# anonymousauthors001/SGS-GNN

Hardware: AMD Instinct MI355X
Metric: sampled edges/sec + training steps/sec, Reddit hybrid 20% sparsity (higher is better)
Workload: dtype f32

## Files before the change

include/sgs_hip.h:

```cpp
#ifndef SGS_HIP_H_
#define SGS_HIP_H_

#include <stddef.h>
#include <stdint.h>

#ifdef __cplusplus
extern "C" {
#endif

#define SGS_ABI_VERSION 1

#define SGS_OK 0
#define SGS_EINVAL (-1)
#define SGS_EWORKSPACE (-2)
#define SGS_EHIP (-3)

typedef void* sgs_stream_t;

int sgs_abi_version(void);
const char* sgs_last_error(void);

int sgs_rng_set_epoch_buffer(const uint64_t* epoch_dev);
int sgs_exp_noise(uint64_t seed, uint64_t stream_id, int64_t E, float* noise, sgs_stream_t stream);
int sgs_dropout_keep(uint64_t seed, uint32_t site, int64_t rows, int64_t cols, float p, uint8_t* keep,
// ... 481 lines not shown
    void* ws;
    size_t ws_bytes;
} SgsGemmTnProblem;
int sgs_gemm_tn_group_supported(int64_t K, int64_t M, int64_t N);
int sgs_gemm_tn_group(const SgsGemmTnProblem* problems, int count, sgs_stream_t stream);

int sgs_er_weight(const int64_t* edge_index, int64_t E, int64_t N, const int32_t* out_ptr, const int32_t* out_dst, int walk_lengths,
                  int walks, uint64_t seed, float* weight, sgs_stream_t stream);

int sgs_adam_max_tensors(void);
int sgs_adam_step(const int64_t* desc_host, int64_t n_tensors, float lr, float beta1, float beta2, float eps, float weight_decay,
                  int maximize, uint32_t* ticket, sgs_stream_t stream);
int sgs_adam_multi_max_tensors(void);
int sgs_adam_step_multi(const int64_t* desc_host, const float* hyper_host, int64_t n_tensors, uint32_t* ticket, float* loss_sum, const float* loss,
                        uint64_t* epoch, sgs_stream_t stream);

size_t sgs_sample_topq_multi_workspace_bytes(int64_t E, int64_t D);
int sgs_sample_topq_multi(int mode, const float* p, const float* prior, double degree_bias_coef, const float* noise, uint64_t seed,
                          uint64_t stream_id0, int64_t D, int64_t E, int64_t q, const int64_t* edge_index, uint8_t* mask, int64_t* sampled_eid,
                          int64_t* sampled_edge_index, float* stats, float* st_weights, void* ws, size_t ws_bytes, sgs_stream_t stream);
size_t sgs_sample_topq_multi_cover_workspace_bytes(int64_t E, int64_t N, int64_t D);
int sgs_sample_topq_multi_cover_group_set(int G);
int sgs_sample_topq_multi_cover(int mode, const float* p, const float* prior, double degree_bias_coef, const float* noise, uint64_t seed,
                                uint64_t stream_id0, int64_t D, int64_t E, int64_t q, const int64_t* edge_index, int64_t N,
                                const int32_t* in_ptr, const int32_t* in_src, const int32_t* in_eid, uint8_t* mask, int64_t* sampled_eid,
                                int64_t* sampled_edge_index, float* stats, float* st_weights, int32_t* cover_info, void* ws, size_t ws_bytes,
                                sgs_stream_t stream);
size_t sgs_graph_filter_multi_workspace_bytes(int64_t E_parent, int64_t N, int64_t D);
int sgs_graph_filter_multi(const int32_t* pin_ptr, const int32_t* pin_src, const int32_t* pin_eid, int64_t E_parent, int64_t N, int64_t D,
                           const uint8_t* mask, const int64_t* sampled_eid, int64_t q, int32_t* in_ptr, int32_t* in_src, int32_t* in_eid,
// ... 82 lines not shown
```

sgs-gnn_amd/csrc/gemm_tn.hip:

```cpp
#include "sgs_common.h"

namespace sgs {
namespace {

using f32x16 = __attribute__((ext_vector_type(16))) float;
constexpr int kUnroll = 8;

__global__ void __launch_bounds__(64) gemm_tn_tile(const float* __restrict__ A, const float* __restrict__ B, int64_t K, int M, int N,
                                                  int ksplit, float* __restrict__ slab) {
    const int lane = threadIdx.x, kh = lane >> 5, l31 = lane & 31;
    const int ti = blockIdx.x, tj = blockIdx.y, s = blockIdx.z;
    const int i = ti * 32 + l31, j = tj * 32 + l31;
    const bool iok = i < M, jok = j < N;
    const int64_t per = ((K + ksplit - 1) / ksplit + 1) & ~int64_t(1);
    const int64_t k0 = s * per, k1 = (k0 + per < K) ? k0 + per : K;
    f32x16 acc;
#pragma unroll
    for (int r = 0; r < 16; ++r) acc[r] = 0.f;
    int64_t k = k0;
    for (; k + 2 * kUnroll <= k1; k += 2 * kUnroll) {
        float a[kUnroll], b[kUnroll];
#pragma unroll
        for (int u = 0; u < kUnroll; ++u) {
            const int64_t kk = k + 2 * u + kh;
// ... 8 lines not shown
        const float a = (iok && kk < k1) ? A[kk * M + i] : 0.f;
        const float b = (jok && kk < k1) ? B[kk * N + j] : 0.f;
        acc = __builtin_amdgcn_mfma_f32_32x32x2f32(a, b, acc, 0, 0, 0);
    }
    float* out = slab + static_cast<int64_t>(s) * M * N;
    if (jok) {
#pragma unroll
        for (int r = 0; r < 16; ++r) {
            const int row = ti * 32 + (r & 3) + 8 * (r >> 2) + 4 * kh;
            if (row < M) out[static_cast<int64_t>(row) * N + j] = acc[r];
        }
    }
}

constexpr int kWgUnroll = 8;
template <int NW>
__device__ __forceinline__ void gemm_tn_wg_tile(const float* __restrict__ A, const float* __restrict__ B, int64_t K, int M, int N,
                                                float* __restrict__ C, int64_t ldc, int ti, int tj) {
    __shared__ float red[NW][16][64];
    const int lane = threadIdx.x & 63, s = threadIdx.x >> 6, kh = lane >> 5, l31 = lane & 31;
    const int i = ti * 32 + l31, j = tj * 32 + l31;
    const bool iok = i < M, jok = j < N;
    const int64_t per = ((K + NW - 1) / NW + 1) & ~int64_t(1);
    const int64_t k0 = s * per, k1 = (k0 + per < K) ? k0 + per : K;
    f32x16 acc;
#pragma unroll
    for (int r = 0; r < 16; ++r) acc[r] = 0.f;
    int64_t k = k0;
    for (; k + 2 * kWgUnroll <= k1; k += 2 * kWgUnroll) {
        float a[kWgUnroll], b[kWgUnroll];
#pragma unroll
        for (int u = 0; u < kWgUnroll; ++u) {
            const int64_t kk = k + 2 * u + kh;
            a[u] = iok ? A[kk * M + i] : 0.f;
// ... 7 lines not shown
        const float a = (iok && kk < k1) ? A[kk * M + i] : 0.f;
        const float b = (jok && kk < k1) ? B[kk * N + j] : 0.f;
        acc = __builtin_amdgcn_mfma_f32_32x32x2f32(a, b, acc, 0, 0, 0);
    }
#pragma unroll
    for (int r = 0; r < 16; ++r) red[s][r][lane] = acc[r];
    __syncthreads();
    if (!jok) return;
    constexpr int RPW = 16 / NW;
#pragma unroll
    for (int q = 0; q < RPW; ++q) {
        const int r = s * RPW + q;
        float sum = 0.f;
#pragma unroll
        for (int z = 0; z < NW; ++z) sum += red[z][r][lane];
        const int row = ti * 32 + (r & 3) + 8 * (r >> 2) + 4 * kh;
        if (row < M) C[static_cast<int64_t>(row) * ldc + j] = sum;
    }
}

template <int NW>
__global__ void __launch_bounds__(64 * NW) gemm_tn_wg(const float* __restrict__ A, const float* __restrict__ B, int64_t K, int M, int N,
                                                     float* __restrict__ C, int64_t ldc) {
    gemm_tn_wg_tile<NW>(A, B, K, M, N, C, ldc, blockIdx.x, blockIdx.y);
}

constexpr int kGroupMax = 8;
struct GemmTnDesc {
    const float* A;
    const float* B;
    float* C;
    int64_t K, ldc;
    int M, N;
    int first_tile, tiles_i;
};
struct GemmTnGroupArgs {
    GemmTnDesc d[kGroupMax];
    int count;
};

template <int NW>
__global__ void __launch_bounds__(64 * NW) gemm_tn_wg_group(GemmTnGroupArgs a) {
    const int t = static_cast<int>(blockIdx.x);
    int pi = 0;
    while (pi + 1 < a.count && t >= a.d[pi + 1].first_tile) ++pi;
    const GemmTnDesc& d = a.d[pi];
    const int local = t - d.first_tile;
    const int tj = local / d.tiles_i, ti = local - tj * d.tiles_i;
    gemm_tn_wg_tile<NW>(d.A, d.B, d.K, d.M, d.N, d.C, d.ldc, ti, tj);
}

__global__ void __launch_bounds__(256) gemm_tn_reduce(const float* __restrict__ slab, int64_t mn, int ksplit, float* __restrict__ C,
                                                      const float* __restrict__ cpart = nullptr, int M = 0, float* __restrict__ colsum = nullptr,
                                                      int N = 0, int64_t ldc = 0, const float* __restrict__ rowscale = nullptr,
                                                      float scale = 1.f, const float* __restrict__ dzpart = nullptr, int nz = 0,
                                                      float* __restrict__ dzsum = nullptr, float* __restrict__ Craw = nullptr,
                                                      float* __restrict__ csraw = nullptr, int csplit = 0) {
    const int64_t i = static_cast<int64_t>(blockIdx.x) * 256 + threadIdx.x;
    if (i >= mn) {
        const int64_t c = i - mn;
        if (dzsum && c == M) {
            float acc = 0.f;
            for (int z = 0; z < nz; ++z) acc += dzpart[z];
            dzsum[0] = acc;
// ... 877 lines not shown
        else              hipLaunchKernelGGL((gemm_tn_wg<2>), grid, dim3(128), 0, stream, A, B, K, static_cast<int>(M), static_cast<int>(N), C, ld);
        SGS_LAUNCH_OK();
        return SGS_OK;
    } else
        hipLaunchKernelGGL(gemm_tn_tile, dim3(cdiv(M, 32), cdiv(N, 32), ks), dim3(64), 0, stream, A, B, K, static_cast<int>(M),
                           static_cast<int>(N), ks, dst);
    if (ks > 1 || strided)
        hipLaunchKernelGGL(gemm_tn_reduce, dim3(cdiv(M * N + (colsum_A ? M : 0), 256)), dim3(256), 0, stream, slab, M * N, n_slabs, C,
                           static_cast<const float*>(colsum_A ? cpart : nullptr), static_cast<int>(M), colsum_A, static_cast<int>(N), ldc);
    SGS_LAUNCH_OK();
    return SGS_OK;
}

int sgs_gemm_tn_group_supported(int64_t K, int64_t M, int64_t N) { return wg_waves(K, M, N); }

int sgs_gemm_tn_group(const SgsGemmTnProblem* problems, int count, sgs_stream_t stream_) {
    hipStream_t stream = static_cast<hipStream_t>(stream_);
    SGS_REQUIRE(count >= 0 && (count == 0 || problems), SGS_EINVAL, "sgs_gemm_tn_group: bad problem list");
    for (int p = 0; p < count; ++p) {
        const SgsGemmTnProblem& q = problems[p];
        SGS_REQUIRE(q.K >= 0 && q.M >= 0 && q.N >= 0 && q.M < (1 << 30) && q.N < (1 << 30), SGS_EINVAL, "sgs_gemm_tn_group: bad sizes");
        SGS_REQUIRE(q.ldc == 0 || q.ldc >= q.N, SGS_EINVAL, "sgs_gemm_tn_group: ldc < N");
        SGS_REQUIRE(q.M == 0 || q.N == 0 || (q.C && (q.K == 0 || (q.A && q.B))), SGS_EINVAL, "sgs_gemm_tn_group: null pointer");
    }
    for (int nw = 16; nw >= 2; nw >>= 1) {
        GemmTnGroupArgs a;
        a.count = 0;
        int tiles = 0;
        auto flush = [&]() {
            if (a.count == 0) return;
            for (int z = a.count; z < kGroupMax; ++z) a.d[z] = a.d[0];
            const dim3 grid(static_cast<unsigned>(tiles));
// ... 16 lines not shown
            tiles += d.tiles_i * static_cast<int>(cdiv(q.N, 32));
            if (a.count == kGroupMax) flush();
        }
        flush();
    }
    SGS_LAUNCH_OK();
    for (int p = 0; p < count; ++p) {
        const SgsGemmTnProblem& q = problems[p];
        if (wg_waves(q.K, q.M, q.N) != 0) continue;
        const int rc = gemm_tn_impl(q.A, q.B, q.K, q.M, q.N, q.C, nullptr, q.ws, q.ws_bytes, stream, q.ldc);
        if (rc != SGS_OK) return rc;
    }
    return SGS_OK;
}

}
```

sgs-gnn_amd/csrc/optim.hip:

```cpp
#include "sgs_common.h"

namespace sgs {
namespace {

constexpr int kAT = 256;
constexpr int kAChunk = 2048;
constexpr int kAMax = 24;

struct AdamDesc {
    float* p;
    const float* g;
    float* m;
    float* v;
    int64_t n;
    float* step;
    const float* gate;
};
struct AdamArgs {
    AdamDesc d[kAMax];
    int chunk_end[kAMax];
    int n_tensors;
    float lr, beta1, beta2, eps, weight_decay;
    int maximize;
    unsigned int* ticket;
};

__global__ void __launch_bounds__(kAT) adam_group(AdamArgs a) {
    __shared__ unsigned int s_last;
    int ti = 0;
    while (static_cast<int>(blockIdx.x) >= a.chunk_end[ti]) ++ti;
    const int chunk = static_cast<int>(blockIdx.x) - (ti ? a.chunk_end[ti - 1] : 0);
    const AdamDesc d = a.d[ti];
    const bool open = d.gate == nullptr || d.gate[0] != 0.f;
    const float t = d.step[0] + 1.0f;
    const double bc1 = 1.0 - exp(static_cast<double>(t) * log(static_cast<double>(a.beta1)));
    const double bc2 = 1.0 - exp(static_cast<double>(t) * log(static_cast<double>(a.beta2)));
    const float step_size = static_cast<float>(static_cast<double>(a.lr) / bc1);
    const float inv_sqrt_bc2 = static_cast<float>(1.0 / sqrt(bc2));
    const float beta1 = a.beta1, beta2 = a.beta2, eps = a.eps, wd = a.weight_decay;
    const int64_t base = static_cast<int64_t>(chunk) * kAChunk;
#pragma unroll
    for (int it = 0; it < kAChunk / kAT; ++it) {
        const int64_t i = base + static_cast<int64_t>(it) * kAT + threadIdx.x;
        if (open && i < d.n) {
            float g = d.g[i];
            if (a.maximize) g = -g;
            const float p = d.p[i];
            if (wd != 0.f) g = fmaf(wd, p, g);
            float m = d.m[i], v = d.v[i];
            m = m + (g - m) * (1.0f - beta1);
            v = beta2 * v + (1.0f - beta2) * g * g;
            const float denom = sqrtf(v) * inv_sqrt_bc2 + eps;
            d.m[i] = m;
            d.v[i] = v;
            d.p[i] = p - step_size * (m / denom);
        }
    }
    __syncthreads();
    if (threadIdx.x == 0) s_last = (atomicAdd(a.ticket, 1u) == gridDim.x - 1) ? 1u : 0u;
    __syncthreads();
    if (s_last) {
        if (static_cast<int>(threadIdx.x) < a.n_tensors) {
            const AdamDesc& dd = a.d[threadIdx.x];
            if (dd.gate == nullptr || dd.gate[0] != 0.f) dd.step[0] += 1.0f;
        }
        if (threadIdx.x == 0) __hip_atomic_store(a.ticket, 0u, __ATOMIC_RELAXED, __HIP_MEMORY_SCOPE_AGENT);
    }
}

constexpr int kAMax2 = 16;
struct AdamState {
    float* m;
    float* v;
    float* step;
    const float* gate;
    float lr, beta1, beta2, eps, wd;
    int maximize;
};
struct AdamDesc2 {
    float* p;
    const float* g;
    int64_t n;
    AdamState s[2];
    int n_states;
};
struct AdamArgs2 {
    AdamDesc2 d[kAMax2];
    int chunk_end[kAMax2];
    int n_tensors;
    unsigned int* ticket;
    float* loss_sum;
    const float* loss;
    unsigned long long* epoch;
};

__global__ void __launch_bounds__(kAT) adam_multi(AdamArgs2 a) {
    __shared__ unsigned int s_last;
    int ti = 0;
    while (static_cast<int>(blockIdx.x) >= a.chunk_end[ti]) ++ti;
    const int chunk = static_cast<int>(blockIdx.x) - (ti ? a.chunk_end[ti - 1] : 0);
    const AdamDesc2& d = a.d[ti];
    bool open[2];
    float step_size[2], inv_sqrt_bc2[2];
#pragma unroll
    for (int q = 0; q < 2; ++q) {
        open[q] = q < d.n_states && (d.s[q].gate == nullptr || d.s[q].gate[0] != 0.f);
        step_size[q] = 0.f;
        inv_sqrt_bc2[q] = 0.f;
        if (q < d.n_states) {
            const float t = d.s[q].step[0] + 1.0f;
            const double bc1 = 1.0 - exp(static_cast<double>(t) * log(static_cast<double>(d.s[q].beta1)));
            const double bc2 = 1.0 - exp(static_cast<double>(t) * log(static_cast<double>(d.s[q].beta2)));
            step_size[q] = static_cast<float>(static_cast<double>(d.s[q].lr) / bc1);
            inv_sqrt_bc2[q] = static_cast<float>(1.0 / sqrt(bc2));
        }
    }
    const int64_t base = static_cast<int64_t>(chunk) * kAChunk;
#pragma unroll
    for (int it = 0; it < kAChunk / kAT; ++it) {
        const int64_t i = base + static_cast<int64_t>(it) * kAT + threadIdx.x;
        if (i < d.n && (open[0] || open[1])) {
            const float g0 = d.g[i];
            float p = d.p[i];
#pragma unroll
            for (int q = 0; q < 2; ++q) {
                if (open[q]) {
                    const AdamState& st = d.s[q];
                    float g = st.maximize ? -g0 : g0;
                    if (st.wd != 0.f) g = fmaf(st.wd, p, g);
                    float m = st.m[i], v = st.v[i];
                    m = m + (g - m) * (1.0f - st.beta1);
                    v = st.beta2 * v + (1.0f - st.beta2) * g * g;
                    const float denom = sqrtf(v) * inv_sqrt_bc2[q] + st.eps;
                    st.m[i] = m;
                    st.v[i] = v;
                    p = p - step_size[q] * (m / denom);
                }
            }
            d.p[i] = p;
        }
    }
    __syncthreads();
    if (threadIdx.x == 0) s_last = (atomicAdd(a.ticket, 1u) == gridDim.x - 1) ? 1u : 0u;
    __syncthreads();
    if (s_last) {
        if (static_cast<int>(threadIdx.x) < 2 * a.n_tensors) {
            const AdamDesc2& dd = a.d[threadIdx.x >> 1];
            const int q = threadIdx.x & 1;
            if (q < dd.n_states && (dd.s[q].gate == nullptr || dd.s[q].gate[0] != 0.f)) {
                dd.s[q].step[0] += 1.0f;
            }
        }
        if (threadIdx.x == 64) {
            if (a.loss_sum && a.loss) a.loss_sum[0] += a.loss[0];
            if (a.epoch) a.epoch[0] += 1ull;
// ... 98 lines not shown
```

sgs-gnn_amd/ops.py:

```python
from __future__ import annotations

import ctypes
import os
from typing import NamedTuple, Optional

import numpy as np
import torch

from . import _lib

SAMPLE_LEARNED, SAMPLE_PRIOR = 0, 1
ACT_NONE, ACT_RELU, ACT_RELU_DROPOUT = 0, 1, 2

_workspaces = {}
_retired_workspaces = []
_pin_workspaces = False


def _need_gpu(*tensors):
    for t in tensors:
        if t is not None and not t.is_cuda:
            raise RuntimeError("sgs_gnn_amd: the SGS hot path runs only on a HIP device (got a CPU tensor); "
                               "there is no CPU fallback")

# ... 93 lines not shown


def new_memo_scope() -> int:
    global _memo_scope
    _memo_scope += 1
    return _memo_scope


def drop_memos(module) -> None:
    for mod in module.modules():
        if getattr(mod, "_lin_cache", None) is not None:
            mod._lin_cache = None


GEMM_TN_LAUNCHES = {"single": 0, "group": 0}
_defer = None
_defer_enabled = True


def set_deferred_weight_grads(on: bool) -> None:
    global _defer_enabled
    _defer_enabled = bool(on)


class deferred_weight_grads:

    def __init__(self, *roots):
        self.roots = roots
        self.producers, self.queue, self.armed, self.prev = {}, [], False, None

    def __enter__(self):
        global _defer
        self.prev = _defer
        if not _defer_enabled:
            return self
        seen, stack = set(), [r.grad_fn for r in self.roots if r.grad_fn is not None]
        prod = self.producers = {}
        while stack:
            fn = stack.pop()
            if fn in seen:
                continue
            seen.add(fn)
            for nxt, _ in fn.next_functions:
                if nxt is None:
# ... 22 lines not shown
        p = node.variable
        if p.grad is not None or getattr(p, "_backward_hooks", None) or getattr(p, "_post_accumulate_grad_hooks", None):
            return None
        return node

    def _enqueue(self, node, dY, x, grad, c_ptr, K, M, N, ldc):
        if not self.armed:
            torch.autograd.Variable._execution_engine.queue_callback(self._flush)
            self.armed = True
        self.queue.append((node, dY, x, grad.data_ptr(), c_ptr, K, M, N, ldc, grad.device.index))

    def _flush(self):
        q, self.queue, self.armed = self.queue, [], False
        if not q:
            return
        L = _lib.lib()
        for node, _, _, base, *_ in q:
            g = node.variable.grad
            if g is None or g.data_ptr() != base:
                raise RuntimeError("sgs_gnn_amd: a deferred weight gradient did not become its parameter's .grad as it was (the values "
                                   "autograd passed on were read before they were written)")
        words = []
        for _, dY, x, _, c_ptr, K, M, N, ldc, _ in q:
            words += [dY.data_ptr(), x.data_ptr(), K, M, N, c_ptr, ldc, 0, 0]
        arr = (ctypes.c_int64 * len(words))(*words)
        dev = q[0][9]
        stream = _raw_stream(dev) if _raw_stream is not None else torch.cuda.current_stream(dev).cuda_stream
        GEMM_TN_LAUNCHES["group"] += 1
        _lib.check(L.sgs_gemm_tn_group(arr, len(q), stream), "sgs_gemm_tn_group")


def _leaf_dw(dY, x, K, M, N, leaf=None, out=None, col0=0):
    L = _lib.lib()
    dW = out if out is not None else torch.empty(M, N, dtype=torch.float32, device=x.device)
    ldc = dW.shape[1]
    c_ptr = _ptr(dW) + 4 * col0
    dY_p, x_p = _ptr(dY, torch.float32), _ptr(x, torch.float32)
    if _defer is not None and leaf is not None and L.sgs_gemm_tn_group_supported(K, M, N) > 0:
        node = _defer._leaf_slot_ok(*leaf)
        if node is not None:
            _defer._enqueue(node, dY, x, dW, c_ptr, K, M, N, ldc)
            return dW
    ws = workspace(L.sgs_gemm_tn_workspace_bytes(K, M, N), x.device)
    GEMM_TN_LAUNCHES["single"] += 1
# ... 2715 lines not shown
```

sgs-gnn_amd/optim.py:

```python
from __future__ import annotations

import ctypes

import torch

from . import _lib, ops


class FusedAdam(torch.optim.Optimizer):
    def __init__(self, params, lr=1e-3, betas=(0.9, 0.999), eps=1e-8, weight_decay=0.0, maximize=False):
        if lr < 0 or eps < 0 or not (0 <= betas[0] < 1) or not (0 <= betas[1] < 1) or weight_decay < 0:
            raise ValueError("FusedAdam: invalid hyper-parameters")
        defaults = dict(lr=lr, betas=betas, eps=eps, weight_decay=weight_decay, maximize=maximize, capturable=True, amsgrad=False,
                        foreach=None, fused=None, differentiable=False)
        super().__init__(params, defaults)
        self._tickets = {}
        self._ticket_pool = None

    def _init_state(self, p):
        if self._ticket_pool is None:
            self._ticket_pool = torch.zeros(64, dtype=torch.int32, device=p.device)
        st = self.state[p]
        if len(st) == 0:
            st["step"] = torch.zeros((), dtype=torch.float32, device=p.device)
# ... 37 lines not shown
                    if self._ticket_pool is not None and len(self._tickets) < self._ticket_pool.numel():
                        i = len(self._tickets)
                        tk = self._tickets[key] = self._ticket_pool[i:i + 1]
                    else:
                        tk = self._tickets[key] = torch.zeros(1, dtype=torch.int32, device=part[0].device)
                arr = (ctypes.c_int64 * len(words))(*words)
                _lib.check(L.sgs_adam_step(arr, len(part), float(group["lr"]), float(b1), float(b2), float(group["eps"]),
                                           float(group["weight_decay"]), int(bool(group["maximize"])), tk.data_ptr(), stream),
                           "sgs_adam_step")
                if not torch.cuda.is_current_stream_capturing():
                    torch.autograd.graph.increment_version(part)
        return loss

    @staticmethod
    @torch.no_grad()
    def step_many(optimizers, tick=None):
        opts = list(optimizers)
        L = _lib.lib()
        order, states = [], {}
        for o in opts:
            if not isinstance(o, FusedAdam):
                raise RuntimeError("FusedAdam.step_many: every optimiser must be a FusedAdam")
            for group in o.param_groups:
                for p in group["params"]:
                    if p.grad is None:
                        continue
                    if id(p) not in states:
                        states[id(p)] = []
                        order.append(p)
                    states[id(p)].append((o, group))
        if any(len(v) > 2 for v in states.values()):
            for o in opts:
                o.step()
            if tick is not None:
                ops.loss_tick(*tick)
            return
        tick_ptrs = (None, None, None)
        if tick is not None:
            loss_sum, loss, epoch = tick
            tick_ptrs = (loss_sum.data_ptr(), loss.detach().reshape(1).data_ptr(), epoch.data_ptr())
        kmax = L.sgs_adam_multi_max_tensors()
        stream = ops._stream()
        first = opts[0]
        if not order:
            if tick is not None:
                ops.loss_tick(*tick)
            return
        for lo in range(0, len(order), kmax):
            part = order[lo:lo + kmax]
            words, hyper = [], []
            for p in part:
                g = p.grad
                if (p.dtype != torch.float32 or g.dtype != torch.float32 or not p.is_cuda or g.is_sparse or not p.is_contiguous()
                        or not g.is_contiguous()):
                    raise RuntimeError("FusedAdam: parameters and gradients must be dense, contiguous float32 HIP tensors")
                w = [p.data_ptr(), g.data_ptr(), p.numel()]
# ... 8 lines not shown
                    h += [0.0] * 6
                words += w
                hyper += h
            key = ("multi", lo, tuple(id(o) for o in opts))
            tk = first._tickets.get(key)
            if tk is None:
                if first._ticket_pool is not None and len(first._tickets) < first._ticket_pool.numel():
                    i = len(first._tickets)
                    tk = first._tickets[key] = first._ticket_pool[i:i + 1]
                else:
                    tk = first._tickets[key] = torch.zeros(1, dtype=torch.int32, device=part[0].device)
            last = lo + kmax >= len(order)
            arr = (ctypes.c_int64 * len(words))(*words)
            hy = (ctypes.c_float * len(hyper))(*hyper)
            tp = tick_ptrs if last else (None, None, None)
            _lib.check(L.sgs_adam_step_multi(arr, hy, len(part), tk.data_ptr(), tp[0], tp[1], tp[2], stream), "sgs_adam_step_multi")
            if not torch.cuda.is_current_stream_capturing():
                torch.autograd.graph.increment_version(part)
```

sgs-gnn_amd/stepgraph.py:

```python
from __future__ import annotations

import ctypes
import gc
import os
import time

import torch

from . import _lib, ops
from .data import Batch
from .sampling import cover_nodes

_DEBUG = os.environ.get("SGS_SG_DEBUG", "")
_PREFETCH = os.environ.get("SGS_SG_PREFETCH", "1") != "0"
_E_ALIGN = 2048


def _capturable(opt) -> bool:
    return all(bool(g.get("capturable", False)) for g in opt.param_groups)


def _opt_signature(optimizers):
    if optimizers is None:
        return None
# ... 438 lines not shown
        self._clear_grads()
        torch.cuda.synchronize()
        c.g1 = torch.cuda.CUDAGraph()
        ops.drop_memos(self.model)
        ops.new_memo_scope()
        if self.dp and self.g3 is None:
            self._capture_g3()
        if not c.sampled:
            if self.dp:
                self._bind_bucket()
            with torch.cuda.graph(c.g1, stream=self.stream, capture_error_mode=self.capture_mode):
                if self.dp:
                    self.sync.flat.zero_()
                out = self.model(batch, batch.edge_index)
                c.loss = _ce(self.criterion, out, batch)
                with ops.deferred_weight_grads(c.loss):
                    c.loss.backward(gradient=self.one)
                self._steps_and_tick((self.optimizers[1],) if (self.optimizers is not None and not self.dp) else (), c.loss)
            c.grads = self._grads()
            c.loss = c.loss.detach()
            self._clear_grads()
            return
        pre, pool = None, None
        if (a.conditional or a.sparse_edge_mlp) and _DEBUG != "fork":
            c.g0 = torch.cuda.CUDAGraph()
            ops.set_rng_epoch_buffer(self.epoch_pre)
            try:
                with ops.workspace_slot(1), torch.cuda.graph(c.g0, stream=self.stream, capture_error_mode=self.capture_mode):
                    pre = sampled_prefix(a, batch, self.q)
            finally:
                ops.set_rng_epoch_buffer(self.epoch_word)
            pool = c.g0.pool()
        with torch.cuda.graph(c.g1, stream=self.stream, pool=pool, capture_error_mode=self.capture_mode):
# ... 2 lines not shown
                                 prefix=pre, gate_publish=(self.epoch_word, self.host_gate))
        pool = c.g1.pool()
        c.cbuf = st.cbuf
        if self.debug_keep:
            c.keep = dict(rsei=st.rsei, eid=st.smp.eid, sampled_edge_index=st.sampled_edge_index,
                          edge_probs_full=st.edge_probs_full.detach(), w=st.edge_probs_for_loss.detach(),
                          learned_out=st.learned_out.detach(),
                          random_out=None if st.random_out is None else st.random_out.detach())
        c.g2l = torch.cuda.CUDAGraph()
        if self.dp:
            self._bind_bucket()
        with torch.cuda.graph(c.g2l, stream=self.stream, pool=pool, capture_error_mode=self.capture_mode):
            if self.dp:
                self.sync.flat.zero_()
            loss_l = learned_loss(a, self.criterion, st, batch)
            with ops.deferred_weight_grads(loss_l):
                loss_l.backward(gradient=self.one, retain_graph=st.random_out is not None)
            if self.dp:
                self.sync.flag.fill_(1.0)
            self._steps_and_tick(tuple(self.optimizers) if (self.optimizers is not None and not self.dp) else (), loss_l)
        c.grads_l = self._grads()
        c.loss_l = loss_l.detach()
        self._clear_grads()
        c.g2r = None
        if st.random_out is not None:
            c.g2r = torch.cuda.CUDAGraph()
            if self.dp:
                self._bind_bucket()
            with torch.cuda.graph(c.g2r, stream=self.stream, pool=pool, capture_error_mode=self.capture_mode):
                if self.dp:
                    self.sync.flat.zero_()
                loss_r = _ce(self.criterion, st.random_out, batch)
                with ops.deferred_weight_grads(loss_r):
                    loss_r.backward(gradient=self.one)
                self._steps_and_tick((self.optimizers[1],) if (self.optimizers is not None and not self.dp) else (), loss_r)
            c.grads_r = self._grads()
            c.loss_r = loss_r.detach()
            self._clear_grads()

    def _steps_and_tick(self, opts, loss) -> None:
        from .optim import FusedAdam
        if opts and all(isinstance(o, FusedAdam) for o in opts):
            FusedAdam.step_many(opts, tick=(self.loss_sum, loss, self.epoch_word))
            return
        for o in opts:
            o.step()
        ops.loss_tick(self.loss_sum, loss, self.epoch_word)

    def _set_grads(self, grads):
        for i, p in enumerate(self.params):
            p.grad = grads.get(i)

    def replay_g1(self, c: _Slot):
        if c.g0 is not None:
            main = torch.cuda.current_stream()
            if self.last_pre is not None:
                main.wait_event(self.last_pre)
            self.epoch_pre.copy_(self.epoch_word)
            c.g0.replay()
# ... 200 lines not shown
```

Measured before the change: 113.0 million.

## Fuse deferred weight-gradient GEMMs with the fused Adam step in one kernel

Deferred weight-gradient GEMM problems are now held back and passed to the optimizer step. A new step_tail kernel computes each gradient tile and applies the Adam update to it in the epilogue, so the gradient is not written and read back before the update. Other tiles take plain Adam chunks in the same grid, and a last-block ticket bumps the step counters, loss sum and epoch. This removes one launch and one round trip of gradients through memory per step. In exchange it adds planning logic with fallbacks to the old path, forces one wave count across all problems, and gives the kernel a large by-value argument block.

```diff
diff --git a/include/sgs_hip.h b/include/sgs_hip.h
--- a/include/sgs_hip.h
+++ b/include/sgs_hip.h
@@ -519,6 +519,11 @@
 int sgs_adam_multi_max_tensors(void);
 int sgs_adam_step_multi(const int64_t* desc_host, const float* hyper_host, int64_t n_tensors, uint32_t* ticket, float* loss_sum, const float* loss,
                         uint64_t* epoch, sgs_stream_t stream);
+int sgs_step_tail_set(int on);
+int sgs_step_tail_max_problems(void);
+int sgs_step_tail_plan(const SgsGemmTnProblem* problems, int count, const int64_t* desc_host, int64_t n_tensors, int nw);
+int sgs_step_tail(const SgsGemmTnProblem* problems, int count, const int64_t* desc_host, const float* hyper_host, int64_t n_tensors,
+                  uint32_t* ticket, float* loss_sum, const float* loss, uint64_t* epoch, int nw, sgs_stream_t stream);
 
 size_t sgs_sample_topq_multi_workspace_bytes(int64_t E, int64_t D);
 int sgs_sample_topq_multi(int mode, const float* p, const float* prior, double degree_bias_coef, const float* noise, uint64_t seed,
diff --git a/sgs-gnn_amd/csrc/adam_update.h b/sgs-gnn_amd/csrc/adam_update.h
--- /dev/null
+++ b/sgs-gnn_amd/csrc/adam_update.h
@@ -0,0 +1,93 @@
+#pragma once
+#include <cstdint>
+
+#include <hip/hip_runtime.h>
+
+namespace sgs {
+
+constexpr int kAMax2 = 16;
+
+struct AdamState {
+    float* m;
+    float* v;
+    float* step;
+    const float* gate;
+    float lr, beta1, beta2, eps, wd;
+    int maximize;
+};
+struct AdamDesc2 {
+    float* p;
+    const float* g;
+    int64_t n;
+    AdamState s[2];
+    int n_states;
+};
+
+__device__ __forceinline__ void adam_update(float g0, float& p, float& m, float& v, float beta1, float beta2, float eps, float wd, bool maximize,
+                                            float step_size, float inv_sqrt_bc2) {
+    float g = maximize ? -g0 : g0;
+    if (wd != 0.f) g = fmaf(wd, p, g);
+    m = m + (g - m) * (1.0f - beta1);
+    v = beta2 * v + (1.0f - beta2) * g * g;
+    const float denom = sqrtf(v) * inv_sqrt_bc2 + eps;
+    p = p - step_size * (m / denom);
+}
+
+__device__ __forceinline__ void adam_bias(float t, float lr, float beta1, float beta2, float& step_size, float& inv_sqrt_bc2) {
+    const double bc1 = 1.0 - exp(static_cast<double>(t) * log(static_cast<double>(beta1)));
+    const double bc2 = 1.0 - exp(static_cast<double>(t) * log(static_cast<double>(beta2)));
+    step_size = static_cast<float>(static_cast<double>(lr) / bc1);
+    inv_sqrt_bc2 = static_cast<float>(1.0 / sqrt(bc2));
+}
+
+struct AdamCoef {
+    bool open[2];
+    float step_size[2], inv_sqrt_bc2[2];
+};
+__device__ __forceinline__ AdamCoef adam_coef(const AdamDesc2& d) {
+    AdamCoef c;
+#pragma unroll
+    for (int q = 0; q < 2; ++q) {
+        c.open[q] = q < d.n_states && (d.s[q].gate == nullptr || d.s[q].gate[0] != 0.f);
+        c.step_size[q] = 0.f;
+        c.inv_sqrt_bc2[q] = 0.f;
+        if (q < d.n_states) adam_bias(d.s[q].step[0] + 1.0f, d.s[q].lr, d.s[q].beta1, d.s[q].beta2, c.step_size[q], c.inv_sqrt_bc2[q]);
+    }
+    return c;
+}
+
+struct AdamElem {
+    float p, m[2], v[2];
+};
+__device__ __forceinline__ AdamElem adam_fetch(const AdamDesc2& d, int64_t i) {
+    AdamElem e;
+    const int q1 = d.n_states > 1 ? 1 : 0;
+    e.p = d.p[i];
+    e.m[0] = d.s[0].m[i];
+    e.v[0] = d.s[0].v[i];
+    e.m[1] = d.s[q1].m[i];
+    e.v[1] = d.s[q1].v[i];
+    return e;
+}
+__device__ __forceinline__ void adam_apply(const AdamDesc2& d, const AdamCoef& c, float g0, AdamElem& e) {
+#pragma unroll
+    for (int q = 0; q < 2; ++q) {
+        if (c.open[q]) {
+            const AdamState& st = d.s[q];
+            adam_update(g0, e.p, e.m[q], e.v[q], st.beta1, st.beta2, st.eps, st.wd, st.maximize != 0, c.step_size[q], c.inv_sqrt_bc2[q]);
+        }
+    }
+}
+__device__ __forceinline__ void adam_store(const AdamDesc2& d, const AdamCoef& c, const AdamElem& e, int64_t i, bool in_range) {
+    if (!in_range) return;
+#pragma unroll
+    for (int q = 0; q < 2; ++q) {
+        if (c.open[q]) {
+            d.s[q].m[i] = e.m[q];
+            d.s[q].v[i] = e.v[q];
+        }
+    }
+    if (c.open[0] || c.open[1]) d.p[i] = e.p;
+}
+
+}
diff --git a/sgs-gnn_amd/csrc/gemm_tn.hip b/sgs-gnn_amd/csrc/gemm_tn.hip
--- a/sgs-gnn_amd/csrc/gemm_tn.hip
+++ b/sgs-gnn_amd/csrc/gemm_tn.hip
@@ -1,4 +1,5 @@
 #include "sgs_common.h"
+#include "adam_update.h"
 
 namespace sgs {
 namespace {
@@ -46,10 +47,15 @@
 }
 
 constexpr int kWgUnroll = 8;
-template <int NW>
+struct NoTileEpilogue {
+    __device__ __forceinline__ void operator()(int, bool, float) const {}
+};
+__device__ __forceinline__ int wg_tile_row(int ti, int r, int kh) { return ti * 32 + (r & 3) + 8 * (r >> 2) + 4 * kh; }
+
+template <int NW, class Epi = NoTileEpilogue>
 __device__ __forceinline__ void gemm_tn_wg_tile(const float* __restrict__ A, const float* __restrict__ B, int64_t K, int M, int N,
-                                                float* __restrict__ C, int64_t ldc, int ti, int tj) {
-    __shared__ float red[NW][16][64];
+                                                float* __restrict__ C, int64_t ldc, int ti, int tj, float (&red)[NW][16][64],
+                                                const Epi& epi = Epi()) {
     const int lane = threadIdx.x & 63, s = threadIdx.x >> 6, kh = lane >> 5, l31 = lane & 31;
     const int i = ti * 32 + l31, j = tj * 32 + l31;
     const bool iok = i < M, jok = j < N;
@@ -87,15 +93,17 @@
         float sum = 0.f;
 #pragma unroll
         for (int z = 0; z < NW; ++z) sum += red[z][r][lane];
-        const int row = ti * 32 + (r & 3) + 8 * (r >> 2) + 4 * kh;
+        const int row = wg_tile_row(ti, r, kh);
         if (row < M) C[static_cast<int64_t>(row) * ldc + j] = sum;
+        epi(q, row < M, sum);
     }
 }
 
 template <int NW>
 __global__ void __launch_bounds__(64 * NW) gemm_tn_wg(const float* __restrict__ A, const float* __restrict__ B, int64_t K, int M, int N,
                                                      float* __restrict__ C, int64_t ldc) {
-    gemm_tn_wg_tile<NW>(A, B, K, M, N, C, ldc, blockIdx.x, blockIdx.y);
+    __shared__ float red[NW][16][64];
+    gemm_tn_wg_tile<NW>(A, B, K, M, N, C, ldc, blockIdx.x, blockIdx.y, red);
 }
 
 constexpr int kGroupMax = 8;
@@ -120,7 +128,116 @@
     const GemmTnDesc& d = a.d[pi];
     const int local = t - d.first_tile;
     const int tj = local / d.tiles_i, ti = local - tj * d.tiles_i;
-    gemm_tn_wg_tile<NW>(d.A, d.B, d.K, d.M, d.N, d.C, d.ldc, ti, tj);
+    __shared__ float red[NW][16][64];
+    gemm_tn_wg_tile<NW>(d.A, d.B, d.K, d.M, d.N, d.C, d.ldc, ti, tj, red);
+}
+
+constexpr int kTailPlainMax = 24;
+struct TailProb {
+    GemmTnDesc g;
+    int64_t off;
+    int adam;
+};
+struct TailPlain {
+    int64_t off, n;
+    int ld, cols;
+    int desc;
+    int chunk_end;
+};
+struct StepTailArgs {
+    TailProb prob[kGroupMax];
+    AdamDesc2 d[kAMax2];
+    TailPlain plain[kTailPlainMax];
+    int n_prob, tiles, n_tensors, n_plain;
+    unsigned int* ticket;
+    float* loss_sum;
+    const float* loss;
+    unsigned long long* epoch;
+};
+static_assert(sizeof(StepTailArgs) <= 4096, "step_tail's by-value argument block must stay under the 4 KB kernel-argument limit");
+
+template <int NW>
+constexpr int tail_iters() { return 2048 / (64 * NW) < 8 ? 2048 / (64 * NW) : 8; }
+
+template <int NW>
+__global__ void __launch_bounds__(64 * NW) step_tail(StepTailArgs a) {
+    __shared__ float red[NW][16][64];
+    unsigned int& s_last = *reinterpret_cast<unsigned int*>(&red[0][0][0]);
+    const int t = static_cast<int>(blockIdx.x);
+    if (t < a.tiles) {
+        int pi = 0;
+        while (pi + 1 < a.n_prob && t >= a.prob[pi + 1].g.first_tile) ++pi;
+        const TailProb& pr = a.prob[pi];
+        const GemmTnDesc& d = pr.g;
+        const int local = t - d.first_tile;
+        const int tj = local / d.tiles_i, ti = local - tj * d.tiles_i;
+        const AdamDesc2& ad = a.d[pr.adam];
+        const AdamCoef c = adam_coef(ad);
+        constexpr int RPW = 16 / NW;
+        const int lane = threadIdx.x & 63, s = threadIdx.x >> 6, kh = lane >> 5;
+        const int j = tj * 32 + (lane & 31), jc = j < d.N ? j : d.N - 1;
+        int64_t idx[RPW];
+        AdamElem e[RPW];
+#pragma unroll
+        for (int q = 0; q < RPW; ++q) {
+            const int row = wg_tile_row(ti, s * RPW + q, kh), rc = row < d.M ? row : d.M - 1;
+            idx[q] = pr.off + static_cast<int64_t>(rc) * d.ldc + jc;
+            e[q] = adam_fetch(ad, idx[q]);
+        }
+        gemm_tn_wg_tile<NW>(d.A, d.B, d.K, d.M, d.N, d.C, d.ldc, ti, tj, red, [&](int q, bool in_range, float sum) {
+            adam_apply(ad, c, sum, e[q]);
+            adam_store(ad, c, e[q], idx[q], in_range);
+        });
+    } else {
+        const int w = t - a.tiles;
+        int bi = 0;
+        while (bi + 1 < a.n_plain && w >= a.plain[bi].chunk_end) ++bi;
+        const TailPlain& b = a.plain[bi];
+        const int chunk = w - (bi ? a.plain[bi - 1].chunk_end : 0);
+        const AdamDesc2& ad = a.d[b.desc];
+        const AdamCoef c = adam_coef(ad);
+        constexpr int IT = tail_iters<NW>(), T = 64 * NW;
+        const int64_t base = static_cast<int64_t>(chunk) * (IT * T);
+        const int64_t last = b.n - 1;
+        const bool strided = b.ld != b.cols;
+        int64_t idx[IT];
+        float g[IT];
+        AdamElem e[IT];
+#pragma unroll
+        for (int it = 0; it < IT; ++it) {
+            const int64_t i = base + static_cast<int64_t>(it) * T + threadIdx.x;
+            const int64_t ic = i < last ? i : last;
+            int64_t x = ic;
+            if (strided) {
+                const uint32_t row = static_cast<uint32_t>(ic) / static_cast<uint32_t>(b.cols);
+                x = static_cast<int64_t>(row) * b.ld + (static_cast<uint32_t>(ic) - row * static_cast<uint32_t>(b.cols));
+            }
+            idx[it] = b.off + x;
+            g[it] = ad.g[idx[it]];
+            e[it] = adam_fetch(ad, idx[it]);
+        }
+#pragma unroll
+        for (int it = 0; it < IT; ++it) {
+            const int64_t i = base + static_cast<int64_t>(it) * T + threadIdx.x;
+            adam_apply(ad, c, g[it], e[it]);
+            adam_store(ad, c, e[it], idx[it], i < b.n);
+        }
+    }
+    __syncthreads();
+    if (threadIdx.x == 0) s_last = (atomicAdd(a.ticket, 1u) == gridDim.x - 1) ? 1u : 0u;
+    __syncthreads();
+    if (s_last) {
+        if (static_cast<int>(threadIdx.x) < 2 * a.n_tensors) {
+            const AdamDesc2& dd = a.d[threadIdx.x >> 1];
+            const int q = threadIdx.x & 1;
+            if (q < dd.n_states && (dd.s[q].gate == nullptr || dd.s[q].gate[0] != 0.f)) dd.s[q].step[0] += 1.0f;
+        }
+        if (threadIdx.x == 64) {
+            if (a.loss_sum && a.loss) a.loss_sum[0] += a.loss[0];
+            if (a.epoch) a.epoch[0] += 1ull;
+        }
+        if (threadIdx.x == 0) __hip_atomic_store(a.ticket, 0u, __ATOMIC_RELAXED, __HIP_MEMORY_SCOPE_AGENT);
+    }
 }
 
 __global__ void __launch_bounds__(256) gemm_tn_reduce(const float* __restrict__ slab, int64_t mn, int ksplit, float* __restrict__ C,
@@ -1028,8 +1145,8 @@
 
 int sgs_gemm_tn_group_supported(int64_t K, int64_t M, int64_t N) { return wg_waves(K, M, N); }
 
-int sgs_gemm_tn_group(const SgsGemmTnProblem* problems, int count, sgs_stream_t stream_) {
-    hipStream_t stream = static_cast<hipStream_t>(stream_);
+static int gemm_tn_group_impl(const SgsGemmTnProblem* problems, int count, hipStream_t stream, int nw_force) {
+    auto wg_waves = [nw_force](int64_t K, int64_t M, int64_t N) { return nw_force && M > 0 && N > 0 ? nw_force : sgs::wg_waves(K, M, N); };
     SGS_REQUIRE(count >= 0 && (count == 0 || problems), SGS_EINVAL, "sgs_gemm_tn_group: bad problem list");
     for (int p = 0; p < count; ++p) {
         const SgsGemmTnProblem& q = problems[p];
@@ -1076,4 +1193,147 @@
     return SGS_OK;
 }
 
-}
+int sgs_gemm_tn_group(const SgsGemmTnProblem* problems, int count, sgs_stream_t stream_) {
+    return gemm_tn_group_impl(problems, count, static_cast<hipStream_t>(stream_), 0);
+}
+
+static int g_step_tail = 1;
+int sgs_step_tail_set(int on) {
+    const int prev = g_step_tail;
+    g_step_tail = on ? 1 : 0;
+    return prev;
+}
+int sgs_step_tail_max_problems(void) { return kGroupMax; }
+
+static int step_tail_plan(const SgsGemmTnProblem* problems, int count, const int64_t* desc, int64_t n_tensors, int nw_force, StepTailArgs* a) {
+    if (count < 1 || count > kGroupMax || n_tensors < 1 || n_tensors > kAMax2) return 0;
+    if (nw_force != 0 && nw_force != 2 && nw_force != 4 && nw_force != 8 && nw_force != 16) return 0;
+    const int64_t* W = desc;
+    for (int64_t i = 0; i < n_tensors; ++i) {
+        if (W[11 * i + 2] < 0) return 0;
+        for (int64_t k = 0; k < i; ++k)
+            if (W[11 * i + 1] == W[11 * k + 1] && W[11 * i + 2] > 0 && W[11 * k + 2] > 0) return 0;
+    }
+    int owner[kAMax2];
+    for (int i = 0; i < kAMax2; ++i) owner[i] = -1;
+    int nw = 0;
+    int64_t tiles = 0;
+    for (int p = 0; p < count; ++p) {
+        const SgsGemmTnProblem& q = problems[p];
+        if (q.K < 0 || q.M <= 0 || q.N <= 0 || q.M >= (1 << 30) || q.N >= (1 << 30) || !q.C || (q.K > 0 && (!q.A || !q.B))) return 0;
+        const int w = nw_force ? nw_force : wg_waves(q.K, q.M, q.N);
+        if (w == 0 || (nw != 0 && w != nw)) return 0;
+        nw = w;
+        const int64_t ldc = q.ldc > 0 ? q.ldc : q.N;
+        if (ldc < q.N || ldc >= (int64_t(1) << 31)) return 0;
+        int k = -1;
+        for (int i = 0; i < n_tensors; ++i) {
+            const float* g = reinterpret_cast<const float*>(W[11 * i + 1]);
+            if (g && q.C >= g && q.C < g + W[11 * i + 2]) { k = i; break; }
+        }
+        if (k < 0 || owner[k] >= 0) return 0;
+        owner[k] = p;
+        const int64_t n = W[11 * k + 2], off = q.C - reinterpret_cast<const float*>(W[11 * k + 1]);
+        if (q.M * ldc != n || off + q.N > ldc) return 0;
+        if (a) {
+            TailProb& t = a->prob[p];
+            t.g.A = q.A; t.g.B = q.B; t.g.C = q.C;
+            t.g.K = q.K; t.g.ldc = ldc;
+            t.g.M = static_cast<int>(q.M); t.g.N = static_cast<int>(q.N);
+            t.g.first_tile = static_cast<int>(tiles);
+            t.g.tiles_i = static_cast<int>(cdiv(q.M, 32));
+            t.off = off;
+            t.adam = k;
+        }
+        tiles += cdiv(q.M, 32) * cdiv(q.N, 32);
+        if (tiles >= (int64_t(1) << 30)) return 0;
+    }
+    const int64_t chunk = 64 * nw * (nw == 16 ? tail_iters<16>() : nw == 8 ? tail_iters<8>() : nw == 4 ? tail_iters<4>() : tail_iters<2>());
+    int np = 0;
+    int64_t chunks = 0;
+    auto add = [&](int desc_i, int64_t off, int64_t rows, int64_t cols, int64_t ld) {
+        if (rows * cols == 0) return true;
+        if (np == kTailPlainMax || (ld != cols && (rows * cols >= (int64_t(1) << 31) || ld >= (int64_t(1) << 31)))) return false;
+        chunks += cdiv(rows * cols, chunk);
+        if (a) {
+            TailPlain& b = a->plain[np];
+            b.off = off; b.n = rows * cols;
+            b.ld = static_cast<int>(ld != cols ? ld : 0); b.cols = static_cast<int>(ld != cols ? cols : 0);
+            b.desc = desc_i;
+            b.chunk_end = static_cast<int>(chunks);
+        }
+        ++np;
+        return chunks < (int64_t(1) << 30);
+    };
+    for (int i = 0; i < n_tensors; ++i) {
+        const int64_t n = W[11 * i + 2];
+        if (owner[i] < 0) {
+            if (!add(i, 0, 1, n, n)) return 0;
+            continue;
+        }
+        const SgsGemmTnProblem& q = problems[owner[i]];
+        const int64_t ldc = q.ldc > 0 ? q.ldc : q.N, off = q.C - reinterpret_cast<const float*>(W[11 * i + 1]);
+        if (!add(i, 0, q.M, off, ldc) || !add(i, off + q.N, q.M, ldc - off - q.N, ldc)) return 0;
+    }
+    if (a) {
+        a->n_prob = count;
+        a->tiles = static_cast<int>(tiles);
+        a->n_tensors = static_cast<int>(n_tensors);
+        a->n_plain = np;
+    }
+    return nw;
+}
+
+int sgs_step_tail_plan(const SgsGemmTnProblem* problems, int count, const int64_t* desc_host, int64_t n_tensors, int nw) {
+    if (count < 0 || n_tensors < 0 || (count > 0 && !problems) || (n_tensors > 0 && !desc_host)) return 0;
+    return step_tail_plan(problems, count, desc_host, n_tensors, nw, nullptr);
+}
+
+int sgs_step_tail(const SgsGemmTnProblem* problems, int count, const int64_t* desc_host, const float* hyper_host, int64_t n_tensors, uint32_t* ticket,
+                  float* loss_sum, const float* loss, uint64_t* epoch, int nw, sgs_stream_t stream_) {
+    hipStream_t stream = static_cast<hipStream_t>(stream_);
+    SGS_REQUIRE(count >= 0 && count <= kGroupMax && n_tensors >= 0 && n_tensors <= kAMax2, SGS_EINVAL,
+                "sgs_step_tail: at most %d problems and %d tensors per call (the argument block travels by value, under 4 KB)", kGroupMax, kAMax2);
+    SGS_REQUIRE(ticket && (count == 0 || problems) && (n_tensors == 0 || (desc_host && hyper_host)), SGS_EINVAL, "sgs_step_tail: null pointer");
+    SGS_REQUIRE(nw == 0 || nw == 2 || nw == 4 || nw == 8 || nw == 16, SGS_EINVAL, "sgs_step_tail: nw must be 0, 2, 4, 8 or 16");
+    StepTailArgs a{};
+    const int NW = g_step_tail ? step_tail_plan(problems, count, desc_host, n_tensors, nw, &a) : 0;
+    if (NW == 0) {
+        const int rc = gemm_tn_group_impl(problems, count, stream, nw);
+        if (rc != SGS_OK) return rc;
+        return sgs_adam_step_multi(desc_host, hyper_host, n_tensors, ticket, loss_sum, loss, epoch, stream_);
+    }
+    for (int i = 0; i < n_tensors; ++i) {
+        const int64_t* w = desc_host + 11 * i;
+        const float* h = hyper_host + 12 * i;
+        AdamDesc2& d = a.d[i];
+        d.p = reinterpret_cast<float*>(w[0]);
+        d.g = reinterpret_cast<const float*>(w[1]);
+        d.n = w[2];
+        d.n_states = w[7] ? 2 : 1;
+        for (int q = 0; q < d.n_states; ++q) {
+            AdamState& st = d.s[q];
+            st.m = reinterpret_cast<float*>(w[3 + 4 * q]);
+            st.v = reinterpret_cast<float*>(w[4 + 4 * q]);
+            st.step = reinterpret_cast<float*>(w[5 + 4 * q]);
+            st.gate = reinterpret_cast<const float*>(w[6 + 4 * q]);
+            st.lr = h[6 * q]; st.beta1 = h[6 * q + 1]; st.beta2 = h[6 * q + 2]; st.eps = h[6 * q + 3]; st.wd = h[6 * q + 4];
+            st.maximize = h[6 * q + 5] != 0.f;
+            SGS_REQUIRE(st.m && st.v && st.step && st.beta1 >= 0.f && st.beta1 < 1.f && st.beta2 >= 0.f && st.beta2 < 1.f && st.eps >= 0.f, SGS_EINVAL,
+                        "sgs_step_tail: bad state %d of descriptor %d", q, i);
+        }
+        SGS_REQUIRE(d.p && d.g && d.n >= 0, SGS_EINVAL, "sgs_step_tail: bad descriptor %d", i);
+    }
+    a.ticket = ticket;
+    a.loss_sum = loss_sum; a.loss = loss; a.epoch = reinterpret_cast<unsigned long long*>(epoch);
+    const int64_t grid_n = static_cast<int64_t>(a.tiles) + (a.n_plain ? a.plain[a.n_plain - 1].chunk_end : 0);
+    const dim3 grid(static_cast<unsigned>(grid_n));
+    if (NW == 16)     hipLaunchKernelGGL((step_tail<16>), grid, dim3(1024), 0, stream, a);
+    else if (NW == 8) hipLaunchKernelGGL((step_tail<8>), grid, dim3(512), 0, stream, a);
+    else if (NW == 4) hipLaunchKernelGGL((step_tail<4>), grid, dim3(256), 0, stream, a);
+    else              hipLaunchKernelGGL((step_tail<2>), grid, dim3(128), 0, stream, a);
+    SGS_LAUNCH_OK();
+    return SGS_OK;
+}
+
+}
diff --git a/sgs-gnn_amd/csrc/optim.hip b/sgs-gnn_amd/csrc/optim.hip
--- a/sgs-gnn_amd/csrc/optim.hip
+++ b/sgs-gnn_amd/csrc/optim.hip
@@ -1,4 +1,5 @@
 #include "sgs_common.h"
+#include "adam_update.h"
 
 namespace sgs {
 namespace {
@@ -32,28 +33,28 @@
     const int chunk = static_cast<int>(blockIdx.x) - (ti ? a.chunk_end[ti - 1] : 0);
     const AdamDesc d = a.d[ti];
     const bool open = d.gate == nullptr || d.gate[0] != 0.f;
-    const float t = d.step[0] + 1.0f;
-    const double bc1 = 1.0 - exp(static_cast<double>(t) * log(static_cast<double>(a.beta1)));
-    const double bc2 = 1.0 - exp(static_cast<double>(t) * log(static_cast<double>(a.beta2)));
-    const float step_size = static_cast<float>(static_cast<double>(a.lr) / bc1);
-    const float inv_sqrt_bc2 = static_cast<float>(1.0 / sqrt(bc2));
-    const float beta1 = a.beta1, beta2 = a.beta2, eps = a.eps, wd = a.weight_decay;
+    float step_size, inv_sqrt_bc2;
+    adam_bias(d.step[0] + 1.0f, a.lr, a.beta1, a.beta2, step_size, inv_sqrt_bc2);
     const int64_t base = static_cast<int64_t>(chunk) * kAChunk;
-#pragma unroll
-    for (int it = 0; it < kAChunk / kAT; ++it) {
-        const int64_t i = base + static_cast<int64_t>(it) * kAT + threadIdx.x;
+    const int64_t last = d.n - 1;
+    float g[kAChunk / kAT], p[kAChunk / kAT], m[kAChunk / kAT], v[kAChunk / kAT];
+#pragma unroll
+    for (int it = 0; it < kAChunk / kAT; ++it) {
+        const int64_t i = base + static_cast<int64_t>(it) * kAT + threadIdx.x;
+        const int64_t ic = i < last ? i : last;
+        g[it] = d.g[ic];
+        p[it] = d.p[ic];
+        m[it] = d.m[ic];
+        v[it] = d.v[ic];
+    }
+#pragma unroll
+    for (int it = 0; it < kAChunk / kAT; ++it) {
+        const int64_t i = base + static_cast<int64_t>(it) * kAT + threadIdx.x;
+        adam_update(g[it], p[it], m[it], v[it], a.beta1, a.beta2, a.eps, a.weight_decay, a.maximize != 0, step_size, inv_sqrt_bc2);
         if (open && i < d.n) {
-            float g = d.g[i];
-            if (a.maximize) g = -g;
-            const float p = d.p[i];
-            if (wd != 0.f) g = fmaf(wd, p, g);
-            float m = d.m[i], v = d.v[i];
-            m = m + (g - m) * (1.0f - beta1);
-            v = beta2 * v + (1.0f - beta2) * g * g;
-            const float denom = sqrtf(v) * inv_sqrt_bc2 + eps;
-            d.m[i] = m;
-            d.v[i] = v;
-            d.p[i] = p - step_size * (m / denom);
+            d.m[i] = m[it];
+            d.v[i] = v[it];
+            d.p[i] = p[it];
         }
     }
     __syncthreads();
@@ -68,22 +69,6 @@
     }
 }
 
-constexpr int kAMax2 = 16;
-struct AdamState {
-    float* m;
-    float* v;
-    float* step;
-    const float* gate;
-    float lr, beta1, beta2, eps, wd;
-    int maximize;
-};
-struct AdamDesc2 {
-    float* p;
-    const float* g;
-    int64_t n;
-    AdamState s[2];
-    int n_states;
-};
 struct AdamArgs2 {
     AdamDesc2 d[kAMax2];
     int chunk_end[kAMax2];
@@ -100,45 +85,23 @@
     while (static_cast<int>(blockIdx.x) >= a.chunk_end[ti]) ++ti;
     const int chunk = static_cast<int>(blockIdx.x) - (ti ? a.chunk_end[ti - 1] : 0);
     const AdamDesc2& d = a.d[ti];
-    bool open[2];
-    float step_size[2], inv_sqrt_bc2[2];
-#pragma unroll
-    for (int q = 0; q < 2; ++q) {
-        open[q] = q < d.n_states && (d.s[q].gate == nullptr || d.s[q].gate[0] != 0.f);
-        step_size[q] = 0.f;
-        inv_sqrt_bc2[q] = 0.f;
-        if (q < d.n_states) {
-            const float t = d.s[q].step[0] + 1.0f;
-            const double bc1 = 1.0 - exp(static_cast<double>(t) * log(static_cast<double>(d.s[q].beta1)));
-            const double bc2 = 1.0 - exp(static_cast<double>(t) * log(static_cast<double>(d.s[q].beta2)));
-            step_size[q] = static_cast<float>(static_cast<double>(d.s[q].lr) / bc1);
-            inv_sqrt_bc2[q] = static_cast<float>(1.0 / sqrt(bc2));
-        }
-    }
+    const AdamCoef c = adam_coef(d);
     const int64_t base = static_cast<int64_t>(chunk) * kAChunk;
-#pragma unroll
-    for (int it = 0; it < kAChunk / kAT; ++it) {
-        const int64_t i = base + static_cast<int64_t>(it) * kAT + threadIdx.x;
-        if (i < d.n && (open[0] || open[1])) {
-            const float g0 = d.g[i];
-            float p = d.p[i];
-#pragma unroll
-            for (int q = 0; q < 2; ++q) {
-                if (open[q]) {
-                    const AdamState& st = d.s[q];
-                    float g = st.maximize ? -g0 : g0;
-                    if (st.wd != 0.f) g = fmaf(st.wd, p, g);
-                    float m = st.m[i], v = st.v[i];
-                    m = m + (g - m) * (1.0f - st.beta1);
-                    v = st.beta2 * v + (1.0f - st.beta2) * g * g;
-                    const float denom = sqrtf(v) * inv_sqrt_bc2[q] + st.eps;
-                    st.m[i] = m;
-                    st.v[i] = v;
-                    p = p - step_size[q] * (m / denom);
-                }
-            }
-            d.p[i] = p;
-        }
+    const int64_t last = d.n - 1;
+    float g[kAChunk / kAT];
+    AdamElem e[kAChunk / kAT];
+#pragma unroll
+    for (int it = 0; it < kAChunk / kAT; ++it) {
+        const int64_t i = base + static_cast<int64_t>(it) * kAT + threadIdx.x;
+        const int64_t ic = i < last ? i : last;
+        g[it] = d.g[ic];
+        e[it] = adam_fetch(d, ic);
+    }
+#pragma unroll
+    for (int it = 0; it < kAChunk / kAT; ++it) {
+        const int64_t i = base + static_cast<int64_t>(it) * kAT + threadIdx.x;
+        adam_apply(d, c, g[it], e[it]);
+        adam_store(d, c, e[it], i, i < d.n);
     }
     __syncthreads();
     if (threadIdx.x == 0) s_last = (atomicAdd(a.ticket, 1u) == gridDim.x - 1) ? 1u : 0u;
diff --git a/sgs-gnn_amd/ops.py b/sgs-gnn_amd/ops.py
--- a/sgs-gnn_amd/ops.py
+++ b/sgs-gnn_amd/ops.py
@@ -131,6 +131,7 @@
 
 
 GEMM_TN_LAUNCHES = {"single": 0, "group": 0}
+STEP_TAIL_CALLS = {"tail": 0}
 _defer = None
 _defer_enabled = True
 
@@ -142,9 +143,10 @@
 
 class deferred_weight_grads:
 
-    def __init__(self, *roots):
+    def __init__(self, *roots, hold=False):
         self.roots = roots
         self.producers, self.queue, self.armed, self.prev = {}, [], False, None
+        self.hold, self.held = bool(hold), []
 
     def __enter__(self):
         global _defer
@@ -197,20 +199,41 @@
         q, self.queue, self.armed = self.queue, [], False
         if not q:
             return
-        L = _lib.lib()
         for node, _, _, base, *_ in q:
             g = node.variable.grad
             if g is None or g.data_ptr() != base:
                 raise RuntimeError("sgs_gnn_amd: a deferred weight gradient did not become its parameter's .grad as it was (the values "
                                    "autograd passed on were read before they were written)")
-        words = []
-        for _, dY, x, _, c_ptr, K, M, N, ldc, _ in q:
-            words += [dY.data_ptr(), x.data_ptr(), K, M, N, c_ptr, ldc, 0, 0]
-        arr = (ctypes.c_int64 * len(words))(*words)
-        dev = q[0][9]
-        stream = _raw_stream(dev) if _raw_stream is not None else torch.cuda.current_stream(dev).cuda_stream
-        GEMM_TN_LAUNCHES["group"] += 1
-        _lib.check(L.sgs_gemm_tn_group(arr, len(q), stream), "sgs_gemm_tn_group")
+        if self.hold:
+            self.held += q
+            return
+        launch_weight_grads(q)
+
+    def take_held(self):
+        q, self.held = self.held, []
+        return q
+
+
+def weight_grad_words(q):
+    words = []
+    for _, dY, x, _, c_ptr, K, M, N, ldc, _ in q:
+        words += [dY.data_ptr(), x.data_ptr(), K, M, N, c_ptr, ldc, 0, 0]
+    return words
+
+
+def launch_weight_grads(q) -> None:
+    if not q:
+        return
+    words = weight_grad_words(q)
+    arr = (ctypes.c_int64 * len(words))(*words)
+    dev = q[0][9]
+    stream = _raw_stream(dev) if _raw_stream is not None else torch.cuda.current_stream(dev).cuda_stream
+    GEMM_TN_LAUNCHES["group"] += 1
+    _lib.check(_lib.lib().sgs_gemm_tn_group(arr, len(q), stream), "sgs_gemm_tn_group")
+
+
+def set_step_tail(on: bool) -> bool:
+    return bool(_lib.lib().sgs_step_tail_set(1 if on else 0))
 
 
 def _leaf_dw(dY, x, K, M, N, leaf=None, out=None, col0=0):
diff --git a/sgs-gnn_amd/optim.py b/sgs-gnn_amd/optim.py
--- a/sgs-gnn_amd/optim.py
+++ b/sgs-gnn_amd/optim.py
@@ -75,9 +75,10 @@
 
     @staticmethod
     @torch.no_grad()
-    def step_many(optimizers, tick=None):
+    def step_many(optimizers, tick=None, pending=None):
         opts = list(optimizers)
         L = _lib.lib()
+        pending = list(pending) if pending else []
         order, states = [], {}
         for o in opts:
             if not isinstance(o, FusedAdam):
@@ -90,6 +91,11 @@
                         states[id(p)] = []
                         order.append(p)
                     states[id(p)].append((o, group))
+        kmax = L.sgs_adam_multi_max_tensors()
+        if pending and (any(len(v) > 2 for v in states.values()) or not order or len(order) > kmax
+                        or len(pending) > L.sgs_step_tail_max_problems()):
+            ops.launch_weight_grads(pending)
+            pending = []
         if any(len(v) > 2 for v in states.values()):
             for o in opts:
                 o.step()
@@ -100,7 +106,6 @@
         if tick is not None:
             loss_sum, loss, epoch = tick
             tick_ptrs = (loss_sum.data_ptr(), loss.detach().reshape(1).data_ptr(), epoch.data_ptr())
-        kmax = L.sgs_adam_multi_max_tensors()
         stream = ops._stream()
         first = opts[0]
         if not order:
@@ -139,6 +144,14 @@
             arr = (ctypes.c_int64 * len(words))(*words)
             hy = (ctypes.c_float * len(hyper))(*hyper)
             tp = tick_ptrs if last else (None, None, None)
-            _lib.check(L.sgs_adam_step_multi(arr, hy, len(part), tk.data_ptr(), tp[0], tp[1], tp[2], stream), "sgs_adam_step_multi")
+            if pending:
+                pw = ops.weight_grad_words(pending)
+                probs = (ctypes.c_int64 * len(pw))(*pw)
+                ops.GEMM_TN_LAUNCHES["group"] += 1
+                ops.STEP_TAIL_CALLS["tail"] += 1
+                _lib.check(L.sgs_step_tail(probs, len(pending), arr, hy, len(part), tk.data_ptr(), tp[0], tp[1], tp[2], 0, stream), "sgs_step_tail")
+                pending = []
+            else:
+                _lib.check(L.sgs_adam_step_multi(arr, hy, len(part), tk.data_ptr(), tp[0], tp[1], tp[2], stream), "sgs_adam_step_multi")
             if not torch.cuda.is_current_stream_capturing():
                 torch.autograd.graph.increment_version(part)
diff --git a/sgs-gnn_amd/stepgraph.py b/sgs-gnn_amd/stepgraph.py
--- a/sgs-gnn_amd/stepgraph.py
+++ b/sgs-gnn_amd/stepgraph.py
@@ -476,9 +476,10 @@
                     self.sync.flat.zero_()
                 out = self.model(batch, batch.edge_index)
                 c.loss = _ce(self.criterion, out, batch)
-                with ops.deferred_weight_grads(c.loss):
+                opts = (self.optimizers[1],) if (self.optimizers is not None and not self.dp) else ()
+                with ops.deferred_weight_grads(c.loss, hold=self._tail_fusable(opts)) as dw:
                     c.loss.backward(gradient=self.one)
-                self._steps_and_tick((self.optimizers[1],) if (self.optimizers is not None and not self.dp) else (), c.loss)
+                self._steps_and_tick(opts, c.loss, pending=dw.take_held())
             c.grads = self._grads()
             c.loss = c.loss.detach()
             self._clear_grads()
@@ -511,11 +512,12 @@
             if self.dp:
                 self.sync.flat.zero_()
             loss_l = learned_loss(a, self.criterion, st, batch)
-            with ops.deferred_weight_grads(loss_l):
+            opts = tuple(self.optimizers) if (self.optimizers is not None and not self.dp) else ()
+            with ops.deferred_weight_grads(loss_l, hold=self._tail_fusable(opts)) as dw:
                 loss_l.backward(gradient=self.one, retain_graph=st.random_out is not None)
             if self.dp:
                 self.sync.flag.fill_(1.0)
-            self._steps_and_tick(tuple(self.optimizers) if (self.optimizers is not None and not self.dp) else (), loss_l)
+            self._steps_and_tick(opts, loss_l, pending=dw.take_held())
         c.grads_l = self._grads()
         c.loss_l = loss_l.detach()
         self._clear_grads()
@@ -528,18 +530,25 @@
                 if self.dp:
                     self.sync.flat.zero_()
                 loss_r = _ce(self.criterion, st.random_out, batch)
-                with ops.deferred_weight_grads(loss_r):
+                opts = (self.optimizers[1],) if (self.optimizers is not None and not self.dp) else ()
+                with ops.deferred_weight_grads(loss_r, hold=self._tail_fusable(opts)) as dw:
                     loss_r.backward(gradient=self.one)
-                self._steps_and_tick((self.optimizers[1],) if (self.optimizers is not None and not self.dp) else (), loss_r)
+                self._steps_and_tick(opts, loss_r, pending=dw.take_held())
             c.grads_r = self._grads()
             c.loss_r = loss_r.detach()
             self._clear_grads()
 
-    def _steps_and_tick(self, opts, loss) -> None:
+    @staticmethod
+    def _tail_fusable(opts) -> bool:
+        from .optim import FusedAdam
+        return bool(opts) and all(isinstance(o, FusedAdam) for o in opts)
+
+    def _steps_and_tick(self, opts, loss, pending=None) -> None:
         from .optim import FusedAdam
         if opts and all(isinstance(o, FusedAdam) for o in opts):
-            FusedAdam.step_many(opts, tick=(self.loss_sum, loss, self.epoch_word))
+            FusedAdam.step_many(opts, tick=(self.loss_sum, loss, self.epoch_word), pending=pending)
             return
+        ops.launch_weight_grads(pending)
         for o in opts:
             o.step()
         ops.loss_tick(self.loss_sum, loss, self.epoch_word)
```

Measured after the change: 114.2 million, median of 6. 1.1% higher.
